# Fabri000/Maze-Solving-Agent-Gymnasium

Hardware: AMD Instinct MI355X
Metric: env steps/sec (whole node) + DQN win-rate, 40x40 r-prim mazes (higher is better)
Workload: dtype int32

## Files before the change

include/mazerl.h:

```cpp
#ifndef MAZERL_H
#define MAZERL_H
#include <stdint.h>

#ifdef __cplusplus
extern "C" {
#endif

#define MZ_OK 0
#define MZ_EINVAL (-1)
#define MZ_EINVAL_SHAPE (-2)
#define MZ_EHIP (-3)
#define MZ_ENOMEM (-4)
#define MZ_EALIGN (-5)

#define MZ_MAX_DIM 127
#define MZ_BANK_MAX_DIMS 64
#define MZ_MAX_CANDIDATES 64
#define MZ_WINDOW 15
#define MZ_WINDOW_BITS 675
#define MZ_WINDOW_WORDS 22

#define MZ_ALGO_RPRIM 0
#define MZ_ALGO_DFS 1
#define MZ_ALGO_PRIMKILL 2
// ... 213 lines not shown
                 const float* reward_dev, double gamma, int32_t b, float* part_dev,
                 uint32_t* ticket_dev, float* loss_dev, float* diff_dev, void* stream);

int mz_head_loss_backward_workspace_floats(int32_t b, int32_t hidden);
int mz_head_loss_backward(const float* grad_dev, const float* diff_dev, const int64_t* action_dev,
                          int32_t b, const float* z2s_dev, int32_t lds, const float* w3s_dev,
                          int32_t hidden, int32_t act, float* dz2_dev, int32_t ldd,
                          float* part_dev, void* stream);

int mz_adamw_groups(float* param_dev, float* exp_avg_dev, float* exp_avg_sq_dev,
                    const float* const* grads_dev, const int64_t* seg_len,
                    const int32_t* seg_group, int32_t nseg, const float* lr_dev, float* step_dev,
                    double beta1, double beta2, double eps, double weight_decay, float max_norm,
                    float* scratch_dev, void* stream);


int mz_ppo_act(const float* logits_dev, int32_t ldl, const float* value_dev, int32_t ldv,
               const float* obs6_dev, const uint32_t* bits_dev, int32_t B, int32_t L, uint64_t seed,
               uint64_t counter, const int32_t* t_dev, float* rec_s6_dev, uint32_t* rec_w_dev,
               int64_t* rec_a_dev, float* rec_lp_dev, float* rec_v_dev, int32_t* act_out_dev,
               void* stream);

int mz_ppo_scan(const double* reward64_dev, const uint8_t* term_dev, const uint8_t* trunc_dev,
                int32_t B, int32_t L, int32_t* t_dev, double* rec_r_dev, int32_t* fin_id_dev,
                int64_t* fin_off_dev, int32_t* fin_len_dev, int32_t* fin_count_dev,
                int64_t* pool_fill_dev, int64_t* pool_total_dev, int64_t* stats_dev,
                void* stream);

int mz_ppo_finish(const double* rec_r_dev, const float* rec_s6_dev, const uint32_t* rec_w_dev,
                  const int64_t* rec_a_dev, const float* rec_lp_dev, const float* rec_v_dev,
                  int32_t B, int32_t L, const int32_t* fin_id_dev, const int64_t* fin_off_dev,
                  const int32_t* fin_len_dev, const int32_t* fin_count_dev, double gamma,
                  int64_t capacity, float* pool_s6_dev, uint32_t* pool_w_dev, int64_t* pool_a_dev,
                  float* pool_lp_dev, float* pool_adv_dev, float* pool_ret_dev, void* stream);

int mz_ppo_head_loss(const float* logits_dev, int32_t ldl, const float* value_dev, int32_t ldv,
                     const int64_t* action_dev, const float* lp_old_dev, const float* adv_dev,
                     const float* ret_dev, const float* coef_dev, int32_t b, float clip,
                     float* scratch_dev, float* loss_dev, float* dlogits_dev, int32_t ldg,
                     float* dvalue_dev, int32_t ldvg, void* stream);


int mz_qact_prepare(const float* fc1_w_dev, const float* fc2_w_dev, uint16_t* w1_hi_dev,
                    uint16_t* w1_lo_dev, uint16_t* w2_hi_dev, uint16_t* w2_lo_dev, void* stream);

int64_t mz_qact_workspace_floats(int32_t n);
int mz_qact(const uint32_t* bits_dev, const float* obs6_dev, const int32_t* rows_dev,
            const int32_t* count_dev, int32_t n, const float* conv_w_dev, const float* conv_b_dev,
            const uint16_t* w1_hi_dev, const uint16_t* w1_lo_dev, const float* b1_dev,
            const uint16_t* w2_hi_dev, const uint16_t* w2_lo_dev, const float* b2_dev,
            const float* w3_dev, const float* b3_dev, int32_t relu, float drop_p, uint64_t seed,
            uint64_t counter, float* h1_dev, int64_t* greedy_dev, float* q_out_dev, void* stream);


int mz_qtab_states(int32_t max_dim, int64_t* rows);

int mz_qtab_act(const float* obs6_dev, int32_t n, int32_t max_dim, const int32_t* table_of_dev,
                int32_t ntables, const uint8_t* active_dev, const double* q_dev,
                int64_t* steps_done_dev, const double* eps_init_dev, const double* eps_final_dev,
                const double* eps_decay_dev, uint64_t seed, uint64_t counter, int32_t* actions_dev,
                int64_t* sidx_dev, void* stream);

int mz_qtab_update(const float* obs6_dev, int32_t n, int32_t max_dim, const int32_t* table_of_dev,
                   int32_t ntables, double* q_dev, const int64_t* sidx_dev,
                   const int32_t* actions_dev, const double* reward64_dev,
                   const uint8_t* terminated_dev, const uint8_t* truncated_dev, double* gamma_dev,
                   const double* lr_dev, const double* eta_dev, double* cum_dev,
                   int64_t* episodes_dev, int64_t* wins_dev, double* td_dev, int32_t episode_end,
                   void* stream);

#ifdef __cplusplus
}
#endif
#endif
```

maze-solving-agent-gymnasium_amd/csrc/mz_api.hip:

```cpp
#include <algorithm>
#include <cmath>
#include <cstdarg>
#include <cstdio>
#include <cstdlib>
#include <cstring>
#include <string>
#include <vector>

#include "../../include/mazerl.h"
#include "mz_common.h"
#include "mz_learner.h"
#include "mz_mcclendon.h"

struct MzHostFallback {
  int cap = 0, gstride = 0;
  uint8_t *grid_h = nullptr, *grid_d = nullptr;
  int32_t *info_h = nullptr, *info_d = nullptr;
  double *prod_h = nullptr, *prod_d = nullptr;
  int32_t *ok_h = nullptr, *ok_d = nullptr;
  int32_t* count_h = nullptr;
  int* count_d = nullptr;
  int32_t* map = nullptr;
};

// ... 1335 lines not shown

int mz_ppo_finish(const double* rec_r_dev, const float* rec_s6_dev, const uint32_t* rec_w_dev,
                  const int64_t* rec_a_dev, const float* rec_lp_dev, const float* rec_v_dev,
                  int32_t B, int32_t L, const int32_t* fin_id_dev, const int64_t* fin_off_dev,
                  const int32_t* fin_len_dev, const int32_t* fin_count_dev, double gamma,
                  int64_t capacity, float* pool_s6_dev, uint32_t* pool_w_dev, int64_t* pool_a_dev,
                  float* pool_lp_dev, float* pool_adv_dev, float* pool_ret_dev, void* stream) {
  if (!rec_r_dev || !rec_s6_dev || !rec_w_dev || !rec_a_dev || !rec_lp_dev || !rec_v_dev ||
      !fin_id_dev || !fin_off_dev || !fin_len_dev || !fin_count_dev || !pool_s6_dev ||
      !pool_w_dev || !pool_a_dev || !pool_lp_dev || !pool_adv_dev || !pool_ret_dev || B < 0 ||
      L < 1 || capacity < 0)
    return fail(MZ_EINVAL, "bad arguments");
  StreamGuard g(stream);
  MzPpoFinish q{rec_r_dev, rec_s6_dev, rec_w_dev, rec_a_dev, rec_lp_dev, rec_v_dev, L, fin_id_dev,
                fin_off_dev, fin_len_dev, fin_count_dev, gamma, capacity, pool_s6_dev, pool_w_dev,
                pool_a_dev, pool_lp_dev, pool_adv_dev, pool_ret_dev};
  MZ_HIP(mz_launch_ppo_finish(q, B, static_cast<hipStream_t>(stream)));
  return MZ_OK;
}

int mz_ppo_head_loss(const float* logits_dev, int32_t ldl, const float* value_dev, int32_t ldv,
                     const int64_t* action_dev, const float* lp_old_dev, const float* adv_dev,
                     const float* ret_dev, const float* coef_dev, int32_t b, float clip,
                     float* scratch_dev, float* loss_dev, float* dlogits_dev, int32_t ldg,
                     float* dvalue_dev, int32_t ldvg, void* stream) {
  if (!logits_dev || !value_dev || !action_dev || !lp_old_dev || !adv_dev || !ret_dev ||
      !coef_dev || !scratch_dev || !loss_dev || !dlogits_dev || !dvalue_dev || b < 0 || ldl < 4 ||
      ldg < 4 || ldv < 1 || ldvg < 1)
    return fail(MZ_EINVAL, "bad arguments");
  StreamGuard g(stream);
  float* w = scratch_dev;
  MzPpoHead q{logits_dev, ldl, value_dev, ldv, action_dev, lp_old_dev, adv_dev, ret_dev, coef_dev,
              b, w, w + b, w + 2 * (size_t)b, w + 6 * (size_t)b, w + 10 * (size_t)b,
              w + 11 * (size_t)b, loss_dev, dlogits_dev, ldg, dvalue_dev, ldvg};
  MZ_HIP(mz_launch_ppo_head(q, clip, static_cast<hipStream_t>(stream)));
  return MZ_OK;
}

int mz_qact_prepare(const float* fc1_w_dev, const float* fc2_w_dev, uint16_t* w1_hi_dev,
                    uint16_t* w1_lo_dev, uint16_t* w2_hi_dev, uint16_t* w2_lo_dev, void* stream) {
  if (!fc1_w_dev || !fc2_w_dev || !w1_hi_dev || !w1_lo_dev || !w2_hi_dev || !w2_lo_dev)
    return fail(MZ_EINVAL, "bad arguments");
  for (const void* p : {(const void*)fc1_w_dev, (const void*)fc2_w_dev, (const void*)w1_hi_dev,
                        (const void*)w1_lo_dev, (const void*)w2_hi_dev, (const void*)w2_lo_dev})
    if (reinterpret_cast<uintptr_t>(p) & 15) return fail(MZ_EINVAL, "weights / images must be 16-B aligned");
  StreamGuard g(stream);
  MZ_HIP(mz_launch_qact_prepare(fc1_w_dev, fc2_w_dev, w1_hi_dev, w1_lo_dev, w2_hi_dev, w2_lo_dev,
                                static_cast<hipStream_t>(stream)));
  return MZ_OK;
}

int64_t mz_qact_workspace_floats(int32_t n) { return n > 0 ? mz_qact_ws_floats(n) : 0; }

int mz_qact(const uint32_t* bits_dev, const float* obs6_dev, const int32_t* rows_dev,
            const int32_t* count_dev, int32_t n, const float* conv_w_dev, const float* conv_b_dev,
            const uint16_t* w1_hi_dev, const uint16_t* w1_lo_dev, const float* b1_dev,
            const uint16_t* w2_hi_dev, const uint16_t* w2_lo_dev, const float* b2_dev,
            const float* w3_dev, const float* b3_dev, int32_t relu, float drop_p, uint64_t seed,
            uint64_t counter, float* h1_dev, int64_t* greedy_dev, float* q_out_dev, void* stream) {
  if (!bits_dev || !obs6_dev || !conv_w_dev || !conv_b_dev || !w1_hi_dev || !w1_lo_dev ||
      !b1_dev || !w2_hi_dev || !w2_lo_dev || !b2_dev || !w3_dev || !b3_dev || !h1_dev || n < 0 ||
      (!greedy_dev && !q_out_dev))
    return fail(MZ_EINVAL, "bad arguments");
  if (count_dev && !rows_dev) return fail(MZ_EINVAL, "a device count needs a row list");
  if (!(drop_p >= 0.0f && drop_p < 1.0f)) return fail(MZ_EINVAL, "dropout p %g", (double)drop_p);
  const uintptr_t al = reinterpret_cast<uintptr_t>(w1_hi_dev) | reinterpret_cast<uintptr_t>(w1_lo_dev) |
                       reinterpret_cast<uintptr_t>(w2_hi_dev) | reinterpret_cast<uintptr_t>(w2_lo_dev) |
                       reinterpret_cast<uintptr_t>(h1_dev) | reinterpret_cast<uintptr_t>(q_out_dev);
  if (al & 15) return fail(MZ_EALIGN, "weight images, h1 and q_out must be 16-byte aligned");
  StreamGuard g(stream);
  const uint64_t k = seed * 0x9E3779B97F4A7C15ull + counter * 0xD1B54A32D192ED03ull + 1;
  MzQAct q{bits_dev, obs6_dev, rows_dev, count_dev, n, conv_w_dev, conv_b_dev, w1_hi_dev,
           w1_lo_dev, b1_dev, w2_hi_dev, w2_lo_dev, b2_dev, w3_dev, b3_dev,
           drop_p > 0.0f ? (uint32_t)(drop_p * 65536.0f + 0.5f) : 0u,
           drop_p > 0.0f ? 1.0f / (1.0f - drop_p) : 1.0f, (uint32_t)(k ^ (k >> 32)), h1_dev,
           greedy_dev, q_out_dev};
  MZ_HIP(mz_launch_qact(q, relu, static_cast<hipStream_t>(stream)));
  return MZ_OK;
}


int mz_qtab_states(int32_t max_dim, int64_t* rows) {
  if (!rows) return fail(MZ_EINVAL, "null argument");
  if (max_dim < 5 || max_dim > MZ_MAX_DIM)
    return fail(MZ_EINVAL, "max_dim %d outside [5, %d]", max_dim, MZ_MAX_DIM);
  const int64_t p = max_dim;
  *rows = 5 * p * p * p * p;
  return MZ_OK;
}

namespace {
int qtab_check(const void* obs6, int32_t n, int32_t max_dim, const void* table_of, int32_t ntables,
               const void* q) {
  if (!q) return fail(MZ_EINVAL, "null Q-table");
  if (!obs6) return fail(MZ_EINVAL, "null observation");
  if (n <= 0) return fail(MZ_EINVAL, "n %d must be >= 1", n);
  if (max_dim < 5 || max_dim > MZ_MAX_DIM)
    return fail(MZ_EINVAL, "max_dim %d outside [5, %d]", max_dim, MZ_MAX_DIM);
  if (ntables <= 0) return fail(MZ_EINVAL, "ntables %d must be >= 1", ntables);
  if (!table_of && ntables != n)
    return fail(MZ_EINVAL, "no table map: ntables %d must equal n %d", ntables, n);
  if (reinterpret_cast<uintptr_t>(q) & 15) return fail(MZ_EALIGN, "Q-table must be 16-byte aligned");
  if (reinterpret_cast<uintptr_t>(obs6) & 7) return fail(MZ_EALIGN, "obs6 must be 8-byte aligned");
  return MZ_OK;
}
}
// ... 44 lines not shown
```

maze-solving-agent-gymnasium_amd/csrc/mz_learner.h:

```cpp
#pragma once
#include "mz_kernels.h"

int mz_stem_chunks(int n);
hipError_t mz_launch_stem_fwd(const uint32_t* bits, const float* obs6, int n, const float* w,
                              const float* b, float drop_p, const uint64_t* rng, uint32_t salt,
                              float* feat, int ld, uint8_t* code, hipStream_t s);
hipError_t mz_launch_stem_bwd(const uint32_t* bits, const uint8_t* code, const float* g, int ld,
                              int n, float drop_p, float* partial, float* dw, float* db,
                              hipStream_t s, uint64_t* advance = nullptr);
#define MZ_OPT_MAX_SEGS 16

hipError_t mz_launch_adamw(float* p, float* m, float* v, const float* const* grads,
                           const int64_t* seg_len, int nseg, const float* lr, float* step, double b1,
                           double b2, double eps, double wd, float clamp, float gscale,
                           int write_grad, hipStream_t s);
hipError_t mz_launch_pair_surrogate(const float* lp_new, const float* lp_old, const float* adv,
                                    int b, float clip, float* part, float* dsum, hipStream_t s);
hipError_t mz_launch_leaky_bf16(uint16_t* x, int64_t n, float slope, hipStream_t s);
hipError_t mz_launch_colsum(const float* g, int n, int m, int ld, float* out, hipStream_t s);
hipError_t mz_launch_replay_gather(const int64_t* idx, int b, int64_t cap, const float* s6,
                                   const uint32_t* sw, const int64_t* a, const float* r,
                                   const float* s6n, const uint32_t* swn, float* o6, uint32_t* ow,
                                   int64_t* oa, float* orw, hipStream_t s);

// ... 50 lines not shown
                                  const int64_t* seg_len, const int32_t* seg_group, int nseg,
                                  const float* lr, float* step, double b1, double b2, double eps,
                                  double wd, float max_norm, float* scratch, hipStream_t s);

struct MzPpoAct {
  const float* logits; int ldl;
  const float* value; int ldv;
  const float* obs6; const uint32_t* bits;
  int B, L;
  uint64_t seed, counter;
  const int32_t* t;
  float* b_s6; uint32_t* b_w; int64_t* b_a; float* b_lp; float* b_v;
  int32_t* act_out;
};
struct MzPpoScan {
  const double* reward64; const uint8_t* term; const uint8_t* trunc;
  int B, L;
  int32_t* t; double* b_r;
  int32_t* fin_id; int64_t* fin_off; int32_t* fin_len; int32_t* fin_count;
  int64_t* pool_fill; int64_t* pool_total; long long* stats;
};
struct MzPpoFinish {
  const double* b_r; const float* b_s6; const uint32_t* b_w; const int64_t* b_a; const float* b_lp;
  const float* b_v; int L;
  const int32_t* fin_id; const int64_t* fin_off; const int32_t* fin_len; const int32_t* fin_count;
  double gamma; int64_t cap;
  float* p_s6; uint32_t* p_w; int64_t* p_a; float* p_lp; float* p_adv; float* p_ret;
};
hipError_t mz_launch_ppo_act(const MzPpoAct& q, hipStream_t s);
hipError_t mz_launch_ppo_scan(const MzPpoScan& q, hipStream_t s);
hipError_t mz_launch_ppo_finish(const MzPpoFinish& q, int max_episodes, hipStream_t s);
struct MzPpoHead {
  const float* logits; int ldl; const float* value; int ldv;
  const int64_t* action; const float* lp_old; const float* adv; const float* ret;
  const float* coef; int b;
  float* lp_new; float* ent; float* p; float* dent; float* part; float* dsum;
  float* loss; float* dlogits; int ldg; float* dvalue; int ldvg;
};
hipError_t mz_launch_ppo_head(const MzPpoHead& q, float clip, hipStream_t s);

struct MzQAct {
  const uint32_t* bits; const float* obs6;
  const int32_t* rows; const int32_t* count; int n;
  const float* conv_w; const float* conv_b;
  const uint16_t* w1h; const uint16_t* w1l; const float* b1;
  const uint16_t* w2h; const uint16_t* w2l; const float* b2;
  const float* w3; const float* b3;
  uint32_t drop_thresh; float drop_scale; uint32_t key;
  float* h1;
  int64_t* greedy; float* q_out;
};
int mz_qact_row_tiles(int n);
int64_t mz_qact_ws_floats(int n);
hipError_t mz_launch_qact(const MzQAct& q, int relu, hipStream_t s);
hipError_t mz_launch_qact_prepare(const float* w1, const float* w2, uint16_t* w1h, uint16_t* w1l,
                                  uint16_t* w2h, uint16_t* w2l, hipStream_t s);

struct MzQtabAct {
  const float* obs6; int n, P;
  const int32_t* table_of; int T;
  const uint8_t* active;
  const double* q; int64_t rows;
  const long long* steps_done;
  const double* eps_init; const double* eps_final; const double* eps_decay;
  uint64_t seed, counter;
  int32_t* actions; int64_t* sidx;
};
struct MzQtabUpd {
  const float* obs6; int n, P;
  const int32_t* table_of; int T;
  double* q; int64_t rows;
  const int64_t* sidx; const int32_t* actions;
  const double* reward64; const uint8_t* terminated; const uint8_t* truncated;
  double* gamma; const double* lr; const double* eta;
  double* cum;
  long long* episodes; long long* wins;
  double* td;
  int episode_end;
};
hipError_t mz_launch_qtab_act(const MzQtabAct& a, long long* steps_done, hipStream_t s);
hipError_t mz_launch_qtab_update(const MzQtabUpd& u, hipStream_t s);
```

maze-solving-agent-gymnasium_amd/csrc/mz_qact.hip:

```cpp
#include <hip/hip_runtime.h>
#include <math.h>
#include <stdint.h>

#include "mz_learner.h"

namespace {

constexpr int WAVE = 64;
constexpr int CONV_OUT = 1568;
constexpr int K1 = 1600;
constexpr int N1 = 1024, N2 = 512;
constexpr int NCH = K1 / 32;
#ifndef MZ_QACT_WAVES
#define MZ_QACT_WAVES 4
#endif
constexpr int QW1 = MZ_QACT_WAVES;
constexpr int T1 = 64 * QW1;
constexpr int RT1 = 64;
constexpr int NT1 = 64 * QW1;
constexpr int TPW = 16 / QW1;
constexpr int NTL1 = N1 / NT1;
constexpr int XPT = 8 / NTL1;
constexpr int PR = 20;
constexpr int AST = 40;
#ifndef MZ_QACT2_ROWS
#define MZ_QACT2_ROWS 64
#endif
constexpr int RT2 = MZ_QACT2_ROWS;
constexpr int MI2 = RT2 / 16;

typedef __attribute__((ext_vector_type(8))) __bf16 frag_ab;
typedef __attribute__((ext_vector_type(4))) float frag_cd;
typedef __attribute__((ext_vector_type(4))) unsigned int u32x4;
typedef __attribute__((ext_vector_type(4))) float f32x4;

__device__ inline uint32_t bf16x2(float lo, float hi) {
  uint32_t r;
  asm("v_cvt_pk_bf16_f32 %0, %1, %2" : "=v"(r) : "v"(lo), "v"(hi));
  return r;
}
__device__ inline float bf16_round(float x) {
  return __uint_as_float(bf16x2(x, 0.0f) << 16);
}
__device__ inline void split2(float x0, float x1, uint32_t& hi, uint32_t& lo) {
  hi = bf16x2(x0, x1);
  const float h0 = __uint_as_float(hi << 16), h1 = __uint_as_float(hi & 0xFFFF0000u);
  lo = bf16x2(x0 - h0, x1 - h1);
}

__device__ inline uint32_t lowbias32(uint32_t x) {
  x ^= x >> 16;
  x *= 0x7FEB352Du;
  x ^= x >> 15;
  x *= 0x846CA68Bu;
  x ^= x >> 16;
// ... 366 lines not shown
    uint32_t* fh = reinterpret_cast<uint32_t*>(ft + (size_t)c * FT_CHUNK);
    uint32_t* fl = fh + RT1 * 16;
#pragma unroll
    for (int tt = 0; tt < TPW; ++tt) {
      fh[il[tt] * 16 + c16] = hi[tt];
      fl[il[tt] * 16 + c16] = lo[tt];
    }
  }
  if (c1 == NCH) {
    uint32_t* fh = reinterpret_cast<uint32_t*>(ft + (size_t)(NCH - 1) * FT_CHUNK);
    for (int i = tid; i < RT1 * 16; i += T1) {
      const int r = i >> 4, k2 = (i & 15) * 2;
      uint32_t hi, lo;
      obs_vals(q, r0, nr, r, k2, hi, lo);
      fh[i] = hi;
      fh[RT1 * 16 + i] = lo;
    }
  }
}

#ifndef MZ_QFC1_WPE
#define MZ_QFC1_WPE 2
#endif
__global__ __launch_bounds__(T1) __attribute__((amdgpu_waves_per_eu(MZ_QFC1_WPE, MZ_QFC1_WPE)))
void k_qfc1(MzQAct q, int row_tiles, const uint16_t* __restrict__ feat) {
  __shared__ __align__(16) uint16_t A[2][QF_CPB][2][RT1 * ARS];
  constexpr int NP = 2 * RT1 * 32 / 8 / T1;
  static_assert(NP * T1 == 2 * RT1 * 32 / 8, "whole 16-B pieces per thread");
  const int tid = threadIdx.x, lane = tid & (WAVE - 1);
  const int w = __builtin_amdgcn_readfirstlane(tid / WAVE);
  const int g4 = lane >> 4, c16 = lane & 15;
  const int b = blockIdx.x, x = b & 7, k = b >> 3;
  const int nt = (x / QF_S) * QF_NTX + k % QF_NTX, rt = (k / QF_NTX) * QF_S + x % QF_S;
  if (rt >= row_tiles) return;
  const int m = q.count ? min(q.n, *q.count) : q.n;
  const int r0 = rt * RT1;
  if (r0 >= m) return;
  const int nr = min(RT1, m - r0);
  const int cq = w;
  const int col0 = nt * NT1 + cq * 64;
  frag_cd acc[4][4];
#pragma unroll
  for (int i = 0; i < 4; ++i)
#pragma unroll
    for (int j = 0; j < 4; ++j) acc[i][j] = frag_cd{0.0f, 0.0f, 0.0f, 0.0f};
  uint4 bh[4], bl[4], nbh[4], nbl[4];
  const auto rs_h = __builtin_amdgcn_make_buffer_rsrc(const_cast<uint16_t*>(q.w1h) + (size_t)nt * NT1 * K1,
                                                      0, NT1 * K1 * 2, 0x00020000);
  const auto rs_l = __builtin_amdgcn_make_buffer_rsrc(const_cast<uint16_t*>(q.w1l) + (size_t)nt * NT1 * K1,
                                                      0, NT1 * K1 * 2, 0x00020000);
  const int boff = (cq * 4 * 64 + lane) * 16;
  auto load_b = [&](int c, uint4* dh, uint4* dl) {
    c = min(c, NCH - 1);
#pragma unroll
    for (int j = 0; j < 4; ++j) {
      const int off = boff + c * (QW1 * 4 * 64 * 16) + j * (64 * 16);
      dh[j] = __builtin_bit_cast(uint4, __builtin_amdgcn_raw_buffer_load_b128(rs_h, off, 0, 0));
      dl[j] = __builtin_bit_cast(uint4, __builtin_amdgcn_raw_buffer_load_b128(rs_l, off, 0, 0));
    }
  };
  const u32x4* fsrc = reinterpret_cast<const u32x4*>(feat + (size_t)rt * NCH * FT_CHUNK);
  frag_ab ah[4], al[4];
  auto fc1_read = [&](int buf, int sub) {
    const uint16_t* Ah = A[buf][sub][0];
    const uint16_t* Al = A[buf][sub][1];
#pragma unroll
    for (int i = 0; i < 4; ++i) {
      const int r = 16 * i + c16;
      ah[i] = __builtin_bit_cast(frag_ab, *reinterpret_cast<const uint4*>(Ah + a_off(r, g4)));
      al[i] = __builtin_bit_cast(frag_ab, *reinterpret_cast<const uint4*>(Al + a_off(r, g4)));
    }
  };
  constexpr int NST = NCH / QF_CPB;
  static_assert(NST * QF_CPB == NCH, "whole stages");
  u32x4 s0[QF_CPB][NP], s1[QF_CPB][NP];
  auto ld = [&](int sg, u32x4 (&r)[QF_CPB][NP]) {
    sg = min(sg, NST - 1);
#pragma unroll
    for (int h = 0; h < QF_CPB; ++h)
#pragma unroll
      for (int k = 0; k < NP; ++k)
        r[h][k] = fsrc[(size_t)(sg * QF_CPB + h) * (FT_CHUNK / 8) + tid + k * T1];
  };
  auto st = [&](int buf, const u32x4 (&r)[QF_CPB][NP]) {
#pragma unroll
    for (int h = 0; h < QF_CPB; ++h)
#pragma unroll
      for (int k = 0; k < NP; ++k) {
        const int pc = tid + k * T1, idx = pc & 255;
        *reinterpret_cast<u32x4*>(A[buf][h][pc >> 8] + a_off(idx >> 2, idx & 3)) = r[h][k];
      }
  };
  auto stage = [&](int sg, u32x4 (&nxt)[QF_CPB][NP]) {
#pragma unroll
    for (int h = 0; h < QF_CPB; ++h) {
      const int c = sg * QF_CPB + h;
      fc1_read(sg & 1, h);
      if ((c & 1) == 0) {
        mfma_x3(ah, al, bh, bl, acc);
        load_b(c + 2, bh, bl);
      } else {
        mfma_x3(ah, al, nbh, nbl, acc);
        load_b(c + 2, nbh, nbl);
      }
      if (QF_CPB > 1) __builtin_amdgcn_sched_barrier(0);
    }
    st((sg + 1) & 1, nxt);
    ld(sg + 3, nxt);
    __syncthreads();
  };
  ld(0, s0);
  st(0, s0);
  ld(1, s1);
  __builtin_amdgcn_sched_barrier(0);
  load_b(0, bh, bl);
  load_b(1, nbh, nbl);
  __builtin_amdgcn_sched_barrier(0);
  ld(2, s0);
  __syncthreads();
  int sg = 0;
  for (; sg + 1 < NST; sg += 2) {
    stage(sg, s1);
    stage(sg + 1, s0);
  }
  if (sg < NST) stage(sg, s1);
#pragma unroll
  for (int j = 0; j < 4; ++j) {
    const int col = col0 + 16 * j + c16;
    const float bb = q.b1[col];
#pragma unroll
    for (int i = 0; i < 4; ++i)
#pragma unroll
      for (int r = 0; r < 4; ++r) {
        const int row = 16 * i + 4 * g4 + r;
        if (row < nr) q.h1[(size_t)(r0 + row) * N1 + col] = leaky(acc[i][j][r] + bb);
      }
  }
}

template <bool RELU>
__global__ __launch_bounds__(512) void k_qact2(MzQAct q) {
  __shared__ __align__(16) uint16_t A[2][1][2][RT2 * ARS];
  __shared__ float part[8][RT2][4];
  const int tid = threadIdx.x, lane = tid & (WAVE - 1);
  const int w = __builtin_amdgcn_readfirstlane(tid / WAVE);
  const int g4 = lane >> 4, c16 = lane & 15;
  const int m = q.count ? min(q.n, *q.count) : q.n;
  const int r0 = blockIdx.x * RT2;
  if (r0 >= m) return;
  const int nr = min(RT2, m - r0);
  const int col0 = 64 * w;

  constexpr int AU = RT2 / 64;
  const int ar = tid >> 3, ak = (tid & 7) * 4;
  struct AV { f32x4 v[AU]; };
  auto load_a = [&](int c) -> AV {
    AV a;
#pragma unroll
    for (int u = 0; u < AU; ++u)
      a.v[u] = *reinterpret_cast<const f32x4*>(q.h1 + (size_t)(r0 + min(ar + 64 * u, nr - 1)) * N1 + 32 * c + ak);
    return a;
  };
  auto store_a = [&](int buf, int sub, const AV& a) {
#pragma unroll
    for (int u = 0; u < AU; ++u) {
      uint32_t h0, l0, h1, l1;
      split2(a.v[u].x, a.v[u].y, h0, l0);
      split2(a.v[u].z, a.v[u].w, h1, l1);
      const int o = a_off(ar + 64 * u, ak >> 3) + (ak & 7);
      uint32_t* ph = reinterpret_cast<uint32_t*>(A[buf][sub][0] + o);
      uint32_t* pl = reinterpret_cast<uint32_t*>(A[buf][sub][1] + o);
      ph[0] = h0; ph[1] = h1;
      pl[0] = l0; pl[1] = l1;
    }
  };
  uint4 bh[4], bl[4], nbh[4], nbl[4];
  const auto rs_h = __builtin_amdgcn_make_buffer_rsrc(const_cast<uint16_t*>(q.w2h), 0, N2 * N1 * 2,
                                                      0x00020000);
  const auto rs_l = __builtin_amdgcn_make_buffer_rsrc(const_cast<uint16_t*>(q.w2l), 0, N2 * N1 * 2,
                                                      0x00020000);
  const int boff = (w * 4 * 64 + lane) * 16;
  auto load_b = [&](int c, uint4* dh, uint4* dl) {
#pragma unroll
    for (int j = 0; j < 4; ++j) {
// ... 138 lines not shown
  for (int p = threadIdx.x; p < NCH * 4 * PREP_ROWS; p += 256) {
    const int c = p / (4 * PREP_ROWS), rr = p % PREP_ROWS;
    const int lane = ((p / PREP_ROWS) & 3) * 16 + sub * PREP_ROWS + rr;
    const float* row = rows + rr * PREP_LD;
    uint32_t hi[4], lo[4];
#pragma unroll
    for (int e = 0; e < 8; e += 2) {
      float v[2];
#pragma unroll
      for (int u = 0; u < 2; ++u) {
        const int f = 32 * c + 8 * (lane >> 4) + e + u;
        const int sf = f < CONV_OUT ? (f & 31) * 49 + (f >> 5) : f;
        v[u] = f < CONV_OUT + 6 ? row[sf] : 0.0f;
      }
      split2(v[0], v[1], hi[e >> 1], lo[e >> 1]);
    }
    const size_t o = ((((size_t)nt * NCH + c) * QW1 + cq) * 4 + j) * 64 + lane;
    reinterpret_cast<uint4*>(w1h)[o] = make_uint4(hi[0], hi[1], hi[2], hi[3]);
    reinterpret_cast<uint4*>(w1l)[o] = make_uint4(lo[0], lo[1], lo[2], lo[3]);
  }
}

__global__ __launch_bounds__(256) void k_qact_prep2(const float* __restrict__ w2,
                                                    uint16_t* __restrict__ w2h,
                                                    uint16_t* __restrict__ w2l) {
  const int o = blockIdx.x * 256 + threadIdx.x;
  if (o >= N2 * N1 / 8) return;
  const int lane = o & 63, j = (o >> 6) & 3, wv = (o >> 8) & 7, c = o >> 11;
  const int r = 64 * wv + 16 * j + (lane & 15), k = 32 * c + 8 * (lane >> 4);
  const float4* src = reinterpret_cast<const float4*>(w2 + (size_t)r * N1 + k);
  const float4 a = src[0], b = src[1];
  uint32_t hi[4], lo[4];
  split2(a.x, a.y, hi[0], lo[0]);
  split2(a.z, a.w, hi[1], lo[1]);
  split2(b.x, b.y, hi[2], lo[2]);
  split2(b.z, b.w, hi[3], lo[3]);
  reinterpret_cast<uint4*>(w2h)[o] = make_uint4(hi[0], hi[1], hi[2], hi[3]);
  reinterpret_cast<uint4*>(w2l)[o] = make_uint4(lo[0], lo[1], lo[2], lo[3]);
}

}

int mz_qact_row_tiles(int n) { return (n + RT1 - 1) / RT1; }

int64_t mz_qact_ws_floats(int n) {
  const int64_t rt = (n + RT1 - 1) / RT1;
  return (int64_t)n * N1 + rt * NCH * FT_CHUNK / 2;
}

#ifndef MZ_QACT_FUSED
#define MZ_QACT_FUSED 0
#endif

hipError_t mz_launch_qact(const MzQAct& q, int relu, hipStream_t s) {
  if (q.n <= 0) return hipSuccess;
  const int rt = (q.n + RT1 - 1) / RT1;
  const int blocks1 = 8 * ((rt + XPT - 1) / XPT);
  if (MZ_QACT_FUSED) {
    if (q.drop_thresh)
      hipLaunchKernelGGL(k_qact1<true>, dim3(blocks1), dim3(T1), 0, s, q, rt);
    else
      hipLaunchKernelGGL(k_qact1<false>, dim3(blocks1), dim3(T1), 0, s, q, rt);
  } else {
    uint16_t* feat = reinterpret_cast<uint16_t*>(q.h1 + (size_t)q.n * N1);
    int groups = 1;
    while (groups < 5 && rt * groups < 512) ++groups;
    if (q.drop_thresh)
      hipLaunchKernelGGL(k_qconv<true>, dim3(rt * groups), dim3(T1), 0, s, q, rt, groups, feat);
    else
      hipLaunchKernelGGL(k_qconv<false>, dim3(rt * groups), dim3(T1), 0, s, q, rt, groups, feat);
    hipLaunchKernelGGL(k_qfc1, dim3(8 * QF_NTX * ((rt + QF_S - 1) / QF_S)), dim3(T1), 0, s, q, rt, feat);
  }
  const int blocks2 = (q.n + RT2 - 1) / RT2;
  if (relu)
    hipLaunchKernelGGL(k_qact2<true>, dim3(blocks2), dim3(512), 0, s, q);
  else
    hipLaunchKernelGGL(k_qact2<false>, dim3(blocks2), dim3(512), 0, s, q);
  return hipGetLastError();
}

hipError_t mz_launch_qact_prepare(const float* w1, const float* w2, uint16_t* w1h, uint16_t* w1l,
                                  uint16_t* w2h, uint16_t* w2l, hipStream_t s) {
  hipLaunchKernelGGL(k_qact_prep1, dim3(N1 / PREP_ROWS), dim3(256), 0, s, w1, w1h, w1l);
  hipLaunchKernelGGL(k_qact_prep2, dim3(N2 * N1 / 8 / 256), dim3(256), 0, s, w2, w2h, w2l);
  return hipGetLastError();
}
```

maze-solving-agent-gymnasium_amd/mazerl/_native.py:

```python
import ctypes as C
import os

from . import _build

c_i32p = C.POINTER(C.c_int32)


class Config(C.Structure):
    _fields_ = [("num_envs", C.c_int32), ("max_dim", C.c_int32), ("toroidal", C.c_int32),
                ("enrich", C.c_int32), ("device", C.c_int32), ("reserved", C.c_int32 * 7)]


class StepOut(C.Structure):
    _fields_ = [("reward", C.c_void_p), ("reward64", C.c_void_p), ("terminated", C.c_void_p),
                ("truncated", C.c_void_p), ("pos", C.c_void_p), ("best_dir", C.c_void_p),
                ("obs6", C.c_void_p), ("window_bits", C.c_void_p), ("window", C.c_void_p),
                ("done_idx", C.c_void_p), ("done_count", C.c_void_p)]


class EnvInfo(C.Structure):
    _fields_ = [(k, C.c_int32) for k in ("n", "start_r", "start_c", "goal_r", "goal_c",
                                         "max_steps", "r", "c", "steps", "invalid_streak",
                                         "nmoves", "last_action", "done")]


MZ_STEP_COUNT_ZEROED = 1
MZ_STEP_AUTORESET = 2
MZ_RNG_PHILOX, MZ_RNG_CPYTHON = 0, 1
MZ_ERRORS = {-1: ValueError, -2: ValueError, -3: RuntimeError, -4: MemoryError, -5: ValueError}

EXPORTS = ["mz_last_error", "mz_device_count", "mz_create", "mz_destroy", "mz_load_mazes",
           "mz_generate", "mz_generate_ex", "mz_generate_state", "mz_reset_all", "mz_reset_list", "mz_reset_done", "mz_step", "mz_step_ex", "mz_direction_mask",
           "mz_act", "mz_step_act", "mz_expand_window", "mz_set_algorithm", "mz_query", "mz_get_grid",
           "mz_difficulty", "mz_maze_complexity", "mz_maze_metrics", "mz_difficulty_batch", "mz_get_meta", "mz_discounted_returns", "mz_q_front",
           "mz_bank_create", "mz_bank_create_dims", "mz_bank_create_ex", "mz_bank_fill", "mz_bank_use",
           "mz_bank_slot_grid", "mz_generate_best", "mz_select_stats", "mz_select_stats_ex",
           "mz_set_debug", "mz_screen_batch", "mz_set_regen_dims",
           "mz_bank_consumed", "mz_state_bytes", "mz_state_save", "mz_state_load",
           "mz_stem_forward", "mz_stem_backward", "mz_stem_backward_ex", "mz_stem_workspace_floats", "mz_adamw_flat",
           "mz_pair_surrogate", "mz_leaky_relu_bf16", "mz_colsum_f32",
           "mz_replay_gather", "mz_host_alloc", "mz_host_free", "mz_q_front_rows", "mz_greedy_rows",
           "mz_trainer_tick", "mz_greedy_scatter", "mz_head_bf16", "mz_replay_push",
           "mz_replay_sample_idx", "mz_q_loss", "mz_q_loss_backward", "mz_head_loss",
           "mz_head_loss_backward", "mz_head_loss_workspace_floats",
           "mz_head_loss_backward_workspace_floats", "mz_adamw_groups",
           "mz_ppo_act", "mz_ppo_scan", "mz_ppo_finish", "mz_ppo_head_loss", "mz_qact_prepare", "mz_qact",
           "mz_qact_workspace_floats", "mz_qtab_states", "mz_qtab_act", "mz_qtab_update"]

_lib = None


def lib_path():
    return _build.LIB


def load(build_if_missing=True):
    global _lib
    if _lib is not None:
        return _lib
    path = os.environ.get("MZ_LIB_OVERRIDE") or _build.LIB
    if not os.path.exists(path):
        if not build_if_missing:
            raise RuntimeError(f"libmazerl.so not built ({path}); run mazerl._build.build()")
        _build.build()
    L = C.CDLL(path)
    vp = C.c_void_p
    L.mz_last_error.restype = C.c_char_p
    L.mz_device_count.argtypes = [c_i32p]
    L.mz_create.argtypes = [C.POINTER(Config), C.POINTER(vp)]
    L.mz_destroy.argtypes = [vp]
    L.mz_load_mazes.argtypes = [vp, vp, C.c_int32, vp, vp, C.c_int32, vp]
    L.mz_generate.argtypes = [vp, vp, C.c_int32, vp, C.c_int32, C.c_int32, C.c_uint64, vp]
    L.mz_generate_ex.argtypes = [vp, vp, C.c_int32, vp, C.c_int32, C.c_int32, C.c_uint64,
                                 C.c_int32, vp]
    L.mz_generate_state.argtypes = [vp, C.c_int32, C.c_int32, C.c_int32, vp, vp]
    L.mz_reset_all.argtypes = [vp, C.POINTER(StepOut), vp]
    L.mz_reset_list.argtypes = [vp, vp, vp, C.c_int32, C.c_int32, C.c_uint64, C.c_uint32,
                                C.POINTER(StepOut), vp]
    L.mz_reset_done.argtypes = [vp, C.c_int32, C.c_uint64, C.c_uint32, C.POINTER(StepOut), vp]
    L.mz_step.argtypes = [vp, vp, C.POINTER(StepOut), vp]
    L.mz_step_ex.argtypes = [vp, vp, C.POINTER(StepOut), C.c_int32, vp]
    L.mz_direction_mask.argtypes = [vp, C.c_int32, vp, vp]
    L.mz_act.argtypes = [vp, vp, C.c_float, vp, C.c_uint64, C.c_uint64, vp, vp]
    L.mz_step_act.argtypes = [vp, vp, C.c_float, vp, C.c_uint64, C.c_uint64, vp,
                              C.POINTER(StepOut), C.c_int32, vp]
    L.mz_expand_window.argtypes = [vp, vp, C.c_int32, vp]
    L.mz_set_algorithm.argtypes = [vp, vp, C.c_int32, vp]
    L.mz_query.argtypes = [vp, C.c_int32, C.POINTER(EnvInfo)]
    L.mz_get_grid.argtypes = [vp, C.c_int32, vp]
    L.mz_get_meta.argtypes = [vp, vp, vp]
    L.mz_discounted_returns.argtypes = [vp, C.c_int32, vp, vp, C.c_int32, C.c_double, vp,
                                        C.c_int32, vp]
    L.mz_difficulty.argtypes = [vp] + [C.c_int32] * 6 + [C.POINTER(C.c_double)]
    L.mz_maze_complexity.argtypes = [vp] + [C.c_int32] * 6 + [C.POINTER(C.c_double)] * 2
    L.mz_maze_metrics.argtypes = [vp, vp, C.c_int32, vp, vp]
    L.mz_difficulty_batch.argtypes = [vp, vp, C.c_int32, vp, vp, vp]
    L.mz_bank_create.argtypes = [vp, C.c_int32, C.c_int32, C.c_uint32]
    L.mz_bank_create_dims.argtypes = [vp, C.c_int32, vp, C.c_int32, C.c_uint32]
    L.mz_bank_create_ex.argtypes = [vp, C.c_int32, vp, C.c_int32, C.c_uint32, C.c_int32]
    L.mz_bank_fill.argtypes = [vp, C.c_int32, C.c_uint64, vp]
# ... 10 lines not shown
    L.mz_bank_consumed.argtypes = [vp, C.c_int32, vp, vp]
    L.mz_state_bytes.argtypes = [vp, C.POINTER(C.c_uint64)]
    L.mz_state_save.argtypes = [vp, vp, C.c_uint64, vp]
    L.mz_state_load.argtypes = [vp, vp, C.c_uint64, vp]
    L.mz_q_front.argtypes = [vp, vp, C.c_int32, vp, vp, C.c_float, C.c_uint64, C.c_uint64, vp,
                             C.c_int32, vp]
    L.mz_q_front_rows.argtypes = [vp, vp, vp, vp, C.c_int32, vp, vp, C.c_float, C.c_uint64,
                                  C.c_uint64, vp, C.c_int32, vp]
    L.mz_greedy_rows.argtypes = [vp, C.c_float, C.c_uint64, C.c_uint64, C.c_int32, vp, vp, vp, vp,
                                 vp]
    L.mz_trainer_tick.argtypes = [vp, vp, vp, C.c_double, C.c_double, C.c_double, vp, vp, vp,
                                  C.c_uint64, C.c_uint64, C.c_int32, vp, vp, vp, vp]
    L.mz_greedy_scatter.argtypes = [vp, C.c_int32, vp, vp, C.c_int32, vp, vp]
    L.mz_head_bf16.argtypes = [vp] * 6 + [C.c_int32] * 9 + [vp] * 7
    L.mz_replay_push.argtypes = [C.c_int32, C.c_int64, C.c_int64] + [vp] * 12 + [C.c_int32,
                                                                                 C.c_int32, vp]
    L.mz_replay_sample_idx.argtypes = [C.c_uint64, C.c_uint64, C.c_int64, C.c_int64, C.c_int64,
                                       vp, C.c_int32, vp]
    L.mz_q_loss.argtypes = [vp, C.c_int32, vp, C.c_int32, vp, C.c_int32, vp, vp, C.c_double,
                            C.c_int32, vp, vp, vp]
    L.mz_q_loss_backward.argtypes = [vp, vp, vp, C.c_int32, C.c_int32, vp, vp]
    L.mz_head_loss.argtypes = [vp, C.c_int32, vp, vp, vp, C.c_int32, vp, vp, C.c_int32, C.c_int32,
                               C.c_int32, vp, vp, C.c_double, C.c_int32, vp, vp, vp, vp, vp]
    L.mz_head_loss_backward.argtypes = [vp, vp, vp, C.c_int32, vp, C.c_int32, vp, C.c_int32,
                                        C.c_int32, vp, C.c_int32, vp, vp]
    L.mz_head_loss_workspace_floats.argtypes = [C.c_int32]
    L.mz_head_loss_backward_workspace_floats.argtypes = [C.c_int32, C.c_int32]
    L.mz_stem_forward.argtypes = [vp, vp, C.c_int32, vp, vp, C.c_float, vp, C.c_uint32, vp,
                                  C.c_int32, vp, vp]
    L.mz_stem_backward.argtypes = [vp, vp, vp, C.c_int32, C.c_int32, C.c_float, vp, vp, vp, vp]
    if hasattr(L, "mz_stem_backward_ex"):
        L.mz_stem_backward_ex.argtypes = [vp, vp, vp, C.c_int32, C.c_int32, C.c_float, vp, vp, vp,
                                          vp, vp]
    L.mz_stem_workspace_floats.argtypes = [C.c_int32]
    L.mz_qact_workspace_floats.argtypes = [C.c_int32]
    L.mz_leaky_relu_bf16.argtypes = [vp, C.c_int64, C.c_float, vp]
    L.mz_colsum_f32.argtypes = [vp, C.c_int32, C.c_int32, C.c_int32, vp, vp]
    L.mz_replay_gather.argtypes = [vp, C.c_int32, C.c_int64] + [vp] * 11
    L.mz_pair_surrogate.argtypes = [vp, vp, vp, C.c_int32, C.c_float, vp, vp, vp]
    L.mz_adamw_flat.argtypes = [vp, vp, vp, vp, vp, C.c_int32, vp, vp, C.c_double, C.c_double,
                                C.c_double, C.c_double, C.c_float, C.c_float, C.c_int32, vp]
    L.mz_adamw_groups.argtypes = [vp, vp, vp, vp, vp, vp, C.c_int32, vp, vp, C.c_double,
                                  C.c_double, C.c_double, C.c_double, C.c_float, vp, vp]
    L.mz_ppo_act.argtypes = [vp, C.c_int32, vp, C.c_int32, vp, vp, C.c_int32, C.c_int32,
                             C.c_uint64, C.c_uint64] + [vp] * 8
    L.mz_ppo_scan.argtypes = [vp, vp, vp, C.c_int32, C.c_int32] + [vp] * 10
    L.mz_ppo_head_loss.argtypes = [vp, C.c_int32, vp, C.c_int32, vp, vp, vp, vp, vp, C.c_int32,
                                   C.c_float, vp, vp, vp, C.c_int32, vp, C.c_int32, vp]
    L.mz_ppo_finish.argtypes = [vp] * 6 + [C.c_int32, C.c_int32] + [vp] * 4 + \
        [C.c_double, C.c_int64] + [vp] * 7
    L.mz_qact_prepare.argtypes = [vp] * 7
    L.mz_qact.argtypes = [vp, vp, vp, vp, C.c_int32] + [vp] * 10 + [C.c_int32, C.c_float,
                                                                   C.c_uint64, C.c_uint64] + [vp] * 4
    L.mz_qtab_states.argtypes = [C.c_int32, C.POINTER(C.c_int64)]
    L.mz_qtab_act.argtypes = [vp, C.c_int32, C.c_int32, vp, C.c_int32, vp, vp, vp, vp, vp, vp,
                              C.c_uint64, C.c_uint64, vp, vp, vp]
    L.mz_qtab_update.argtypes = [vp, C.c_int32, C.c_int32, vp, C.c_int32] + [vp] * 13 + \
        [C.c_int32, vp]
    L.mz_host_alloc.argtypes = [C.c_uint64, C.c_int32, C.POINTER(vp), C.POINTER(vp)]
    L.mz_host_free.argtypes = [vp]
    for f in EXPORTS:
        if f != "mz_last_error" and (hasattr(L, f) or not os.environ.get("MZ_LIB_OVERRIDE")):
            getattr(L, f).restype = C.c_int
    L.mz_qact_workspace_floats.restype = C.c_int64
    _lib = L
    return L


def check(rc):
    if rc != 0:
        msg = load().mz_last_error().decode(errors="replace")
        raise MZ_ERRORS.get(rc, RuntimeError)(f"libmazerl error {rc}: {msg}")
    return rc
```

profiles/exp_qact_checksum.py:

```python
#!/usr/bin/env python3
import hashlib
import json
import os
import sys

ROOT = os.path.dirname(os.path.dirname(os.path.abspath(__file__)))
sys.path.insert(0, os.path.join(ROOT, "maze-solving-agent-gymnasium_amd"))

import torch


def main():
    from mazerl.agents.nets import QNet
    from mazerl.agents.qact import QAct
    dev = torch.device("cuda", 0)
    torch.manual_seed(0)
    h = hashlib.sha256()
    for variant in ("ddqn", "dqn"):
        net = QNet(variant=variant).to(dev)
        qa = QAct(net, seed=1)
        g = torch.Generator(device=dev).manual_seed(0)
        n = 65536
        bits = torch.randint(0, 2**31 - 1, (n, 22), generator=g, device=dev, dtype=torch.int32)
        obs6 = torch.rand(n, 6, generator=g, device=dev)
        rows = torch.randperm(n, generator=g, device=dev)[:28180].to(torch.int32).contiguous()
        count = torch.tensor([28180], dtype=torch.int32, device=dev)
        for train in (True, False):
            net.train(train)
            q = qa(obs6, bits)
            h.update(q.cpu().numpy().tobytes())
            qo = torch.zeros(rows.numel(), 4, device=dev)
            gr = torch.zeros(n, dtype=torch.int64, device=dev)
            qa.rows_greedy(obs6, bits, rows, count, gr, q_out=qo)
            h.update(qo.cpu().numpy().tobytes())
            h.update(gr.cpu().numpy().tobytes())
    print(json.dumps({"lib": os.environ.get("MZ_LIB_OVERRIDE", "default"),
                      "q_checksum": h.hexdigest()[:16]}), flush=True)


if __name__ == "__main__":
    main()
```

profiles/summarize_qact_pmc.py:

```python
#!/usr/bin/env python3
import collections
import csv
import glob
import json
import os
import statistics
import sys


def short(name):
    name = name.replace("(anonymous namespace)::", "")
    if name.startswith("void "):
        name = name[5:]
    return name.split("(")[0]


def main(d):
    vals = collections.defaultdict(lambda: collections.defaultdict(list))
    for sub in ("a", "b", "fetch", "write"):
        for f in glob.glob(os.path.join(d, sub, "**", "*counter_collection.csv"), recursive=True):
            for r in csv.DictReader(open(f)):
                k = (short(r["Kernel_Name"]), int(r["Grid_Size"]))
                vals[k][r["Counter_Name"]].append(float(r["Counter_Value"]))
    dur = collections.defaultdict(list)
    for f in glob.glob(os.path.join(d, "kt", "**", "*kernel_trace.csv"), recursive=True):
        for r in csv.DictReader(open(f)):
            g = int(r["Grid_Size_X"]) * int(r["Grid_Size_Y"]) * int(r["Grid_Size_Z"])
            dur[(short(r["Kernel_Name"]), g)].append(int(r["End_Timestamp"]) - int(r["Start_Timestamp"]))
    out = {}
    for k, cs in sorted(vals.items()):
        if not k[0].startswith("k_q"):
            continue
        m = {c: statistics.mean(v) for c, v in cs.items()}
        rec = {"grid": k[1], "counters": {c: round(v, 1) for c, v in m.items()}}
        if k in dur:
            rec["kernel_trace_avg_us"] = round(statistics.mean(dur[k]) / 1e3, 2)
        if "SQ_VALU_MFMA_BUSY_CYCLES" in m and "GRBM_GUI_ACTIVE" in m:
            rec["mfma_busy"] = round(m["SQ_VALU_MFMA_BUSY_CYCLES"] / (m["GRBM_GUI_ACTIVE"] / 8 * 1024), 3)
        if "SQ_INSTS_VALU" in m and m.get("SQ_INSTS_MFMA"):
            rec["valu_per_mfma"] = round(m["SQ_INSTS_VALU"] / m["SQ_INSTS_MFMA"], 2)
        if "FETCH_SIZE" in m and "WRITE_SIZE" in m:
            rec["hbm_mb"] = round((2 * m["FETCH_SIZE"] + m["WRITE_SIZE"]) * 1024 / 1e6, 1)
        out[f"{k[0]} grid {k[1]}"] = rec
    print(json.dumps(out, indent=1))


if __name__ == "__main__":
    main(sys.argv[1])
```

Baseline: 2.004 billion.

## Add wide 128-row fc1 kernel for Q-action batches above threshold

After: 2.002 billion (median of 3 runs). No clear change (-0.1%).

```diff
diff --git a/include/mazerl.h b/include/mazerl.h
--- a/include/mazerl.h
+++ b/include/mazerl.h
@@ -289,6 +289,8 @@
             const float* w3_dev, const float* b3_dev, int32_t relu, float drop_p, uint64_t seed,
             uint64_t counter, float* h1_dev, int64_t* greedy_dev, float* q_out_dev, void* stream);
 
+int mz_qact_fc1_rows(int32_t rows);
+
 
 int mz_qtab_states(int32_t max_dim, int64_t* rows);
 
diff --git a/maze-solving-agent-gymnasium_amd/csrc/mz_api.hip b/maze-solving-agent-gymnasium_amd/csrc/mz_api.hip
--- a/maze-solving-agent-gymnasium_amd/csrc/mz_api.hip
+++ b/maze-solving-agent-gymnasium_amd/csrc/mz_api.hip
@@ -1411,6 +1411,11 @@
 
 int64_t mz_qact_workspace_floats(int32_t n) { return n > 0 ? mz_qact_ws_floats(n) : 0; }
 
+int mz_qact_fc1_rows(int32_t rows) {
+  if (mz_qact_set_fc1_rows(rows) != 0) return fail(MZ_EINVAL, "fc1 rows %d: 0, 64 or 128", rows);
+  return MZ_OK;
+}
+
 int mz_qact(const uint32_t* bits_dev, const float* obs6_dev, const int32_t* rows_dev,
             const int32_t* count_dev, int32_t n, const float* conv_w_dev, const float* conv_b_dev,
             const uint16_t* w1_hi_dev, const uint16_t* w1_lo_dev, const float* b1_dev,
diff --git a/maze-solving-agent-gymnasium_amd/csrc/mz_learner.h b/maze-solving-agent-gymnasium_amd/csrc/mz_learner.h
--- a/maze-solving-agent-gymnasium_amd/csrc/mz_learner.h
+++ b/maze-solving-agent-gymnasium_amd/csrc/mz_learner.h
@@ -126,6 +126,7 @@
 };
 int mz_qact_row_tiles(int n);
 int64_t mz_qact_ws_floats(int n);
+int mz_qact_set_fc1_rows(int rows);
 hipError_t mz_launch_qact(const MzQAct& q, int relu, hipStream_t s);
 hipError_t mz_launch_qact_prepare(const float* w1, const float* w2, uint16_t* w1h, uint16_t* w1l,
                                   uint16_t* w2h, uint16_t* w2l, hipStream_t s);
diff --git a/maze-solving-agent-gymnasium_amd/csrc/mz_qact.hip b/maze-solving-agent-gymnasium_amd/csrc/mz_qact.hip
--- a/maze-solving-agent-gymnasium_amd/csrc/mz_qact.hip
+++ b/maze-solving-agent-gymnasium_amd/csrc/mz_qact.hip
@@ -1,6 +1,8 @@
 #include <hip/hip_runtime.h>
 #include <math.h>
 #include <stdint.h>
+
+#include <atomic>
 
 #include "mz_learner.h"
 
@@ -473,6 +475,15 @@
   const int boff = (cq * 4 * 64 + lane) * 16;
   auto load_b = [&](int c, uint4* dh, uint4* dl) {
     c = min(c, NCH - 1);
+#ifdef MZ_QPROBE_HALF_B
+#pragma unroll
+    for (int j = 0; j < 2; ++j) {
+      const int off = boff + c * (QW1 * 4 * 64 * 16) + j * (64 * 16);
+      dh[j] = dh[j + 2] = __builtin_bit_cast(uint4, __builtin_amdgcn_raw_buffer_load_b128(rs_h, off, 0, 0));
+      dl[j] = dl[j + 2] = __builtin_bit_cast(uint4, __builtin_amdgcn_raw_buffer_load_b128(rs_l, off, 0, 0));
+    }
+    return;
+#endif
 #pragma unroll
     for (int j = 0; j < 4; ++j) {
       const int off = boff + c * (QW1 * 4 * 64 * 16) + j * (64 * 16);
@@ -551,6 +562,108 @@
     const float bb = q.b1[col];
 #pragma unroll
     for (int i = 0; i < 4; ++i)
+#pragma unroll
+      for (int r = 0; r < 4; ++r) {
+        const int row = 16 * i + 4 * g4 + r;
+        if (row < nr) q.h1[(size_t)(r0 + row) * N1 + col] = leaky(acc[i][j][r] + bb);
+      }
+  }
+}
+
+constexpr int RTW = 2 * RT1;
+constexpr int QWIDE_INFLIGHT = 8;
+static_assert(MZ_QA_SWZ && ARS == 32, "k_qwide's DMA pieces are whole 64-B rows");
+static_assert(QW1 == 4 && NCH % 2 == 0, "k_qwide: 4 waves, chunk loop unrolled by two");
+
+__global__ __launch_bounds__(T1) __attribute__((amdgpu_waves_per_eu(2, 2)))
+void k_qwide(MzQAct q, int row_tiles, const uint16_t* __restrict__ feat) {
+  __shared__ __align__(16) uint16_t A[2][2][2][RT1 * ARS];
+  const int tid = threadIdx.x, lane = tid & (WAVE - 1);
+  const int w = __builtin_amdgcn_readfirstlane(tid / WAVE);
+  const int g4 = lane >> 4, c16 = lane & 15;
+  const int b = blockIdx.x, x = b & 7;
+  const int nt = x / XPT, wt = (b >> 3) * XPT + x % XPT;
+  if (2 * wt >= row_tiles) return;
+  const int m = q.count ? min(q.n, *q.count) : q.n;
+  const int r0 = wt * RTW;
+  if (r0 >= m) return;
+  const int nr = min(RTW, m - r0);
+  const int col0 = nt * NT1 + w * 64;
+  frag_cd acc[8][4];
+#pragma unroll
+  for (int i = 0; i < 8; ++i)
+#pragma unroll
+    for (int j = 0; j < 4; ++j) acc[i][j] = frag_cd{0.0f, 0.0f, 0.0f, 0.0f};
+  uint4 bh[4], bl[4], nbh[4], nbl[4];
+  const auto rs_h = __builtin_amdgcn_make_buffer_rsrc(const_cast<uint16_t*>(q.w1h) + (size_t)nt * NT1 * K1,
+                                                      0, NT1 * K1 * 2, 0x00020000);
+  const auto rs_l = __builtin_amdgcn_make_buffer_rsrc(const_cast<uint16_t*>(q.w1l) + (size_t)nt * NT1 * K1,
+                                                      0, NT1 * K1 * 2, 0x00020000);
+  const int boff = (w * 4 * 64 + lane) * 16;
+  auto load_b = [&](int c, uint4* dh, uint4* dl) {
+    c = min(c, NCH - 1);
+#pragma unroll
+    for (int j = 0; j < 4; ++j) {
+      const int off = boff + c * (QW1 * 4 * 64 * 16) + j * (64 * 16);
+      dh[j] = __builtin_bit_cast(uint4, __builtin_amdgcn_raw_buffer_load_b128(rs_h, off, 0, 0));
+      dl[j] = __builtin_bit_cast(uint4, __builtin_amdgcn_raw_buffer_load_b128(rs_l, off, 0, 0));
+    }
+  };
+  const int ft = min(2 * wt + (w >> 1), row_tiles - 1);
+  const uint16_t* gsrc = feat + (size_t)ft * NCH * FT_CHUNK + (w & 1) * (RT1 * 32) + (lane >> 2) * 32 +
+                         8 * ((lane & 3) ^ ((4 - g4) & 3));
+  auto dma = [&](int c) {
+    const uint16_t* g = gsrc + (size_t)min(c, NCH - 1) * FT_CHUNK;
+    uint16_t* l = A[c & 1][w >> 1][w & 1];
+#pragma unroll
+    for (int k = 0; k < 4; ++k)
+      __builtin_amdgcn_global_load_lds((__attribute__((address_space(1))) const void*)(g + k * 16 * 32),
+                                       (__attribute__((address_space(3))) void*)(l + k * 16 * ARS), 16, 0, 0);
+  };
+  frag_ab ah[4], al[4];
+  auto a_read = [&](int buf, int t) {
+    const uint16_t* Ah = A[buf][t][0];
+    const uint16_t* Al = A[buf][t][1];
+#pragma unroll
+    for (int i = 0; i < 4; ++i) {
+      const int r = 16 * i + c16;
+      ah[i] = __builtin_bit_cast(frag_ab, *reinterpret_cast<const uint4*>(Ah + a_off(r, g4)));
+      al[i] = __builtin_bit_cast(frag_ab, *reinterpret_cast<const uint4*>(Al + a_off(r, g4)));
+    }
+  };
+  auto wait_dma_and_barrier = [&]() {
+    __builtin_amdgcn_sched_barrier(0);
+    __builtin_amdgcn_s_waitcnt(0x0F70 | QWIDE_INFLIGHT);
+    asm volatile("s_waitcnt lgkmcnt(0)" ::: "memory");
+    __builtin_amdgcn_s_barrier();
+    asm volatile("" ::: "memory");
+  };
+  auto step = [&](int c, uint4 (&xh)[4], uint4 (&xl)[4]) {
+    a_read(c & 1, 0);
+    mfma_x3<4>(ah, al, xh, xl, *reinterpret_cast<frag_cd(*)[4][4]>(&acc[0]));
+    a_read(c & 1, 1);
+    dma(c + 1);
+    __builtin_amdgcn_sched_barrier(0);
+    mfma_x3<4>(ah, al, xh, xl, *reinterpret_cast<frag_cd(*)[4][4]>(&acc[4]));
+    load_b(c + 2, xh, xl);
+    wait_dma_and_barrier();
+  };
+  load_b(0, bh, bl);
+  __builtin_amdgcn_sched_barrier(0);
+  dma(0);
+  __builtin_amdgcn_sched_barrier(0);
+  load_b(1, nbh, nbl);
+  wait_dma_and_barrier();
+  for (int c = 0; c < NCH; c += 2) {
+    step(c, bh, bl);
+    step(c + 1, nbh, nbl);
+  }
+#pragma unroll
+  for (int j = 0; j < 4; ++j) {
+    const int col = col0 + 16 * j + c16;
+    const float bb = q.b1[col];
+#pragma unroll
+    for (int i = 0; i < 8; ++i)
 #pragma unroll
       for (int r = 0; r < 4; ++r) {
         const int row = 16 * i + 4 * g4 + r;
@@ -795,6 +908,22 @@
 #define MZ_QACT_FUSED 0
 #endif
 
+static std::atomic<int> g_fc1_rows{0};
+#ifndef MZ_QWIDE_MIN_ROWS
+#define MZ_QWIDE_MIN_ROWS 16384
+#endif
+
+int mz_qact_set_fc1_rows(int rows) {
+  if (rows != 0 && rows != RT1 && rows != RTW) return -1;
+  g_fc1_rows.store(rows, std::memory_order_relaxed);
+  return 0;
+}
+
+static int qact_fc1_rows(int n) {
+  const int r = g_fc1_rows.load(std::memory_order_relaxed);
+  return r ? r : (n >= MZ_QWIDE_MIN_ROWS ? RTW : RT1);
+}
+
 hipError_t mz_launch_qact(const MzQAct& q, int relu, hipStream_t s) {
   if (q.n <= 0) return hipSuccess;
   const int rt = (q.n + RT1 - 1) / RT1;
@@ -812,7 +941,12 @@
       hipLaunchKernelGGL(k_qconv<true>, dim3(rt * groups), dim3(T1), 0, s, q, rt, groups, feat);
     else
       hipLaunchKernelGGL(k_qconv<false>, dim3(rt * groups), dim3(T1), 0, s, q, rt, groups, feat);
-    hipLaunchKernelGGL(k_qfc1, dim3(8 * QF_NTX * ((rt + QF_S - 1) / QF_S)), dim3(T1), 0, s, q, rt, feat);
+    if (qact_fc1_rows(q.n) == RTW) {
+      const int wt = (rt + 1) / 2;
+      hipLaunchKernelGGL(k_qwide, dim3(8 * ((wt + XPT - 1) / XPT)), dim3(T1), 0, s, q, rt, feat);
+    } else {
+      hipLaunchKernelGGL(k_qfc1, dim3(8 * QF_NTX * ((rt + QF_S - 1) / QF_S)), dim3(T1), 0, s, q, rt, feat);
+    }
   }
   const int blocks2 = (q.n + RT2 - 1) / RT2;
   if (relu)
diff --git a/maze-solving-agent-gymnasium_amd/mazerl/_native.py b/maze-solving-agent-gymnasium_amd/mazerl/_native.py
--- a/maze-solving-agent-gymnasium_amd/mazerl/_native.py
+++ b/maze-solving-agent-gymnasium_amd/mazerl/_native.py
@@ -45,7 +45,7 @@
            "mz_head_loss_backward", "mz_head_loss_workspace_floats",
            "mz_head_loss_backward_workspace_floats", "mz_adamw_groups",
            "mz_ppo_act", "mz_ppo_scan", "mz_ppo_finish", "mz_ppo_head_loss", "mz_qact_prepare", "mz_qact",
-           "mz_qact_workspace_floats", "mz_qtab_states", "mz_qtab_act", "mz_qtab_update"]
+           "mz_qact_workspace_floats", "mz_qact_fc1_rows", "mz_qtab_states", "mz_qtab_act", "mz_qtab_update"]
 
 _lib = None
 
@@ -162,6 +162,8 @@
     L.mz_qact_prepare.argtypes = [vp] * 7
     L.mz_qact.argtypes = [vp, vp, vp, vp, C.c_int32] + [vp] * 10 + [C.c_int32, C.c_float,
                                                                    C.c_uint64, C.c_uint64] + [vp] * 4
+    if hasattr(L, "mz_qact_fc1_rows") or not os.environ.get("MZ_LIB_OVERRIDE"):
+        L.mz_qact_fc1_rows.argtypes = [C.c_int32]
     L.mz_qtab_states.argtypes = [C.c_int32, C.POINTER(C.c_int64)]
     L.mz_qtab_act.argtypes = [vp, C.c_int32, C.c_int32, vp, C.c_int32, vp, vp, vp, vp, vp, vp,
                               C.c_uint64, C.c_uint64, vp, vp, vp]
diff --git a/profiles/exp_qact_checksum.py b/profiles/exp_qact_checksum.py
--- a/profiles/exp_qact_checksum.py
+++ b/profiles/exp_qact_checksum.py
@@ -13,6 +13,9 @@
 def main():
     from mazerl.agents.nets import QNet
     from mazerl.agents.qact import QAct
+    if len(sys.argv) > 1:
+        from mazerl import _native as N
+        N.check(N.load().mz_qact_fc1_rows(int(sys.argv[1])))
     dev = torch.device("cuda", 0)
     torch.manual_seed(0)
     h = hashlib.sha256()
@@ -35,6 +38,7 @@
             h.update(qo.cpu().numpy().tobytes())
             h.update(gr.cpu().numpy().tobytes())
     print(json.dumps({"lib": os.environ.get("MZ_LIB_OVERRIDE", "default"),
+                      "fc1_rows": int(sys.argv[1]) if len(sys.argv) > 1 else 0,
                       "q_checksum": h.hexdigest()[:16]}), flush=True)
 
 
diff --git a/profiles/exp_qwide.py b/profiles/exp_qwide.py
--- /dev/null
+++ b/profiles/exp_qwide.py
@@ -0,0 +1,61 @@
+#!/usr/bin/env python3
+import json
+import os
+import sys
+
+ROOT = os.path.dirname(os.path.dirname(os.path.abspath(__file__)))
+sys.path.insert(0, os.path.join(ROOT, "maze-solving-agent-gymnasium_amd"))
+import torch
+
+
+def main(mode="sweep", *sizes):
+    from mazerl import _native as N
+    from mazerl.agents.nets import QNet
+    from mazerl.agents.qact import QAct
+    dev = torch.device("cuda", 0)
+    torch.manual_seed(0)
+    net = QNet(variant="ddqn").to(dev)
+    net.train(True)
+    qa = QAct(net, seed=1)
+    lib = N.load()
+    overrides = (64, 128) if hasattr(lib, "mz_qact_fc1_rows") else (0,)
+    st = torch.cuda.current_stream(dev)
+
+    def select(rows):
+        if rows:
+            N.check(lib.mz_qact_fc1_rows(rows))
+
+    def timed(fn, iters=30, warm=5):
+        for _ in range(warm):
+            fn()
+        e0, e1 = torch.cuda.Event(enable_timing=True), torch.cuda.Event(enable_timing=True)
+        e0.record(st)
+        for _ in range(iters):
+            fn()
+        e1.record(st)
+        torch.cuda.synchronize()
+        return round(e0.elapsed_time(e1) / iters * 1e3, 1)
+
+    out = {"lib": os.environ.get("MZ_LIB_OVERRIDE", "default"), "mode": mode}
+    for n in [int(s) for s in sizes] or [65536]:
+        g = torch.Generator(device=dev).manual_seed(0)
+        bits = torch.randint(0, 2**31 - 1, (n, 22), generator=g, device=dev, dtype=torch.int32)
+        obs6 = torch.rand(n, 6, generator=g, device=dev)
+        m = int(0.43 * n)
+        rows = torch.randperm(n, generator=g, device=dev)[:m].to(torch.int32).contiguous()
+        count = torch.tensor([m], dtype=torch.int32, device=dev)
+        greedy = torch.zeros(n, dtype=torch.int64, device=dev)
+        for r in overrides:
+            select(r)
+            if mode == "prof":
+                out[f"all_{n}_fc1rows{r}_us"] = timed(lambda: qa.greedy(obs6, bits, out=greedy), 10, 3)
+                continue
+            out[f"all_{n}_fc1rows{r}_us"] = [timed(lambda: qa.greedy(obs6, bits, out=greedy))
+                                             for _ in range(2)]
+            out[f"list_{m}_of_{n}_fc1rows{r}_us"] = [
+                timed(lambda: qa.rows_greedy(obs6, bits, rows, count, greedy)) for _ in range(2)]
+    print(json.dumps(out), flush=True)
+
+
+if __name__ == "__main__":
+    main(*sys.argv[1:])
diff --git a/profiles/summarize_qact_pmc.py b/profiles/summarize_qact_pmc.py
--- a/profiles/summarize_qact_pmc.py
+++ b/profiles/summarize_qact_pmc.py
@@ -39,6 +39,8 @@
             rec["mfma_busy"] = round(m["SQ_VALU_MFMA_BUSY_CYCLES"] / (m["GRBM_GUI_ACTIVE"] / 8 * 1024), 3)
         if "SQ_INSTS_VALU" in m and m.get("SQ_INSTS_MFMA"):
             rec["valu_per_mfma"] = round(m["SQ_INSTS_VALU"] / m["SQ_INSTS_MFMA"], 2)
+        if "SQ_INSTS_VMEM" in m and m.get("SQ_INSTS_MFMA"):
+            rec["vmem_per_mfma"] = round(m["SQ_INSTS_VMEM"] / m["SQ_INSTS_MFMA"], 4)
         if "FETCH_SIZE" in m and "WRITE_SIZE" in m:
             rec["hbm_mb"] = round((2 * m["FETCH_SIZE"] + m["WRITE_SIZE"]) * 1024 / 1e6, 1)
         out[f"{k[0]} grid {k[1]}"] = rec
```
